# MasterBin-IIAU/UNINEXT

Measured on AMD Instinct MI355X. Metric: frames/sec COCO det+seg R50 1333x800 (MSDeformAttn hot path); MSDeformAttn HBM GB/s, higher is better.
Workload: dtype f32

## Files before the change

include/msda_hip.h:

```cpp
#ifndef MSDA_HIP_H_
#define MSDA_HIP_H_

#include <stddef.h>
#include <stdint.h>

#ifdef __cplusplus
extern "C" {
#endif

#define MSDA_HIP_ABI_VERSION 2

#define MSDA_ERR_NULL_POINTER (-1)
#define MSDA_ERR_BAD_DIMS (-2)
#define MSDA_ERR_TOO_LARGE (-3)
#define MSDA_ERR_BAD_VARIANT (-4)
#define MSDA_ERR_UNSUPPORTED (-5)

int msda_hip_abi_version(void);
const char* msda_hip_last_error(void);

int msda_hip_forward_f32(const float* value, const int64_t* spatial_shapes,
                         const int64_t* level_start_index, const float* sampling_loc,
                         const float* attn_weight, int batch, int spatial_size, int num_heads,
                         int channels, int num_levels, int num_query, int num_point,
                         float* output, void* stream);

int msda_hip_forward_f64(const double* value, const int64_t* spatial_shapes,
                         const int64_t* level_start_index, const double* sampling_loc,
                         const double* attn_weight, int batch, int spatial_size, int num_heads,
                         int channels, int num_levels, int num_query, int num_point,
                         double* output, void* stream);

int msda_hip_backward_f32(const float* grad_output, const float* value,
                          const int64_t* spatial_shapes, const int64_t* level_start_index,
                          const float* sampling_loc, const float* attn_weight, int batch,
                          int spatial_size, int num_heads, int channels, int num_levels,
                          int num_query, int num_point, float* grad_value,
                          float* grad_sampling_loc, float* grad_attn_weight, void* stream);

size_t msda_hip_backward_workspace_bytes(int batch, int spatial_size, int num_heads, int channels, int num_levels,
                                         int num_query, int num_point);
int msda_hip_backward_ws_f32(const float* grad_output, const float* value,
                             const int64_t* spatial_shapes, const int64_t* level_start_index,
                             const float* sampling_loc, const float* attn_weight, int batch,
                             int spatial_size, int num_heads, int channels, int num_levels,
                             int num_query, int num_point, float* grad_value,
                             float* grad_sampling_loc, float* grad_attn_weight, void* workspace,
                             size_t workspace_bytes, void* stream);

int msda_hip_backward_f64(const double* grad_output, const double* value,
                          const int64_t* spatial_shapes, const int64_t* level_start_index,
                          const double* sampling_loc, const double* attn_weight, int batch,
                          int spatial_size, int num_heads, int channels, int num_levels,
                          int num_query, int num_point, double* grad_value,
                          double* grad_sampling_loc, double* grad_attn_weight, void* stream);

int msda_hip_forward_fused_f32(const float* value, const int64_t* spatial_shapes,
                               const int64_t* level_start_index, const float* reference_points, int ref_dim,
                               const float* sampling_offsets, const float* attn_logits, int batch,
                               int spatial_size, int num_heads, int channels, int num_levels, int num_query,
                               int num_point, float* output, void* stream);

int msda_hip_forward_fused_hm_f32(const float* value_head_major, const int64_t* spatial_shapes,
                                  const int64_t* level_start_index, const float* reference_points, int ref_dim,
                                  const float* sampling_offsets, const float* attn_logits, int batch, int spatial_size,
                                  int num_heads, int channels, int num_levels, int num_query, int num_point,
                                  float* output, void* stream);

int msda_hip_prologue_f32(const int64_t* spatial_shapes, const float* reference_points, int ref_dim,
                          const float* sampling_offsets, const float* attn_logits, int batch, int num_heads,
                          int num_levels, int num_query, int num_point, float* sampling_loc, float* attn_weight,
                          void* stream);
int msda_hip_prologue_backward_f32(const int64_t* spatial_shapes, const float* reference_points, int ref_dim,
                                   const float* sampling_offsets, const float* attn_weight,
                                   const float* grad_sampling_loc, const float* grad_attn_weight, int batch,
                                   int num_heads, int num_levels, int num_query, int num_point,
                                   float* grad_sampling_offsets, float* grad_attn_logits,
                                   float* grad_reference_points, void* stream);

int msda_host_forward_f32(const float* value, const int64_t* spatial_shapes, const int64_t* level_start_index,
                          const float* sampling_loc, const float* attn_weight, int batch, int spatial_size,
                          int num_heads, int channels, int num_levels, int num_query, int num_point,
                          float* output, int num_threads);
int msda_host_forward_f64(const double* value, const int64_t* spatial_shapes, const int64_t* level_start_index,
                          const double* sampling_loc, const double* attn_weight, int batch, int spatial_size,
                          int num_heads, int channels, int num_levels, int num_query, int num_point,
                          double* output, int num_threads);
int msda_host_backward_f32(const float* grad_output, const float* value, const int64_t* spatial_shapes,
                           const int64_t* level_start_index, const float* sampling_loc, const float* attn_weight,
                           int batch, int spatial_size, int num_heads, int channels, int num_levels, int num_query,
                           int num_point, float* grad_value, float* grad_sampling_loc, float* grad_attn_weight,
                           int num_threads);
int msda_host_backward_f64(const double* grad_output, const double* value, const int64_t* spatial_shapes,
                           const int64_t* level_start_index, const double* sampling_loc, const double* attn_weight,
                           int batch, int spatial_size, int num_heads, int channels, int num_levels, int num_query,
                           int num_point, double* grad_value, double* grad_sampling_loc, double* grad_attn_weight,
                           int num_threads);

int msda_host_last_num_threads(void);

int msda_hip_set_variant(int which, int variant);
int msda_hip_get_variant(int which);
const char* msda_hip_variant_name(int which, int variant);

const char* msda_hip_last_kernel(int which);

#define MSDA_CTX_GEOMETRY_CHECKED 1u
#define MSDA_CTX_DETERMINISTIC 2u
void msda_hip_set_call_context(int call_site, unsigned flags);
int msda_hip_forward_locality(double* far_fraction);
void msda_hip_reset_call_site(int call_site);

#ifdef __cplusplus
}
#endif
#endif
```

uninext_amd/_lib.py:

```python
import ctypes
import os

_HERE = os.path.dirname(os.path.abspath(__file__))
LIB_PATH = os.environ.get("MSDA_HIP_LIB") or os.path.join(_HERE, "lib", "libmsda_hip.so")

ABI_VERSION = 2

i, p, s, f = ctypes.c_int, ctypes.c_void_p, ctypes.c_char_p, ctypes.c_float
u, z, ll, dp = ctypes.c_uint, ctypes.c_size_t, ctypes.c_longlong, ctypes.POINTER(ctypes.c_double)
_FWD = [p, p, p, p, p, i, i, i, i, i, i, i, p]
_BWD = [p, p, p, p, p, p, i, i, i, i, i, i, i, p, p, p]

_SIGNATURES = {
    "msda_hip.h": {
        "msda_hip_abi_version": (i, []),
        "msda_hip_last_error": (s, []),
        "msda_hip_forward_f32": (i, _FWD + [p]),
        "msda_hip_forward_f64": (i, _FWD + [p]),
        "msda_hip_backward_f32": (i, _BWD + [p]),
        "msda_hip_backward_workspace_bytes": (z, [i, i, i, i, i, i, i]),
        "msda_hip_backward_ws_f32": (i, _BWD + [p, z, p]),
        "msda_hip_backward_f64": (i, _BWD + [p]),
        "msda_hip_forward_fused_f32": (i, [p, p, p, p, i, p, p, i, i, i, i, i, i, i, p, p]),
        "msda_hip_forward_fused_hm_f32": (i, [p, p, p, p, i, p, p, i, i, i, i, i, i, i, p, p]),
        "msda_hip_prologue_f32": (i, [p, p, i, p, p, i, i, i, i, i, p, p, p]),
        "msda_hip_prologue_backward_f32": (i, [p, p, i, p, p, p, p, i, i, i, i, i, p, p, p, p]),
        "msda_host_forward_f32": (i, _FWD + [i]),
        "msda_host_forward_f64": (i, _FWD + [i]),
        "msda_host_backward_f32": (i, _BWD + [i]),
        "msda_host_backward_f64": (i, _BWD + [i]),
        "msda_host_last_num_threads": (i, []),
        "msda_hip_set_variant": (i, [i, i]),
        "msda_hip_get_variant": (i, [i]),
        "msda_hip_variant_name": (s, [i, i]),
        "msda_hip_last_kernel": (s, [i]),
        "msda_hip_set_call_context": (None, [i, u]),
        "msda_hip_forward_locality": (i, [dp]),
        "msda_hip_reset_call_site": (None, [i]),
    },
    "dynmask_hip.h": {
        "dynmask_hip_forward_f32": (i, [p, p, p, p, i, i, i, i, i, i, p, p]),
        "aligned_bilinear_hip_f32": (i, [p, i, i, i, i, p, p]),
        "dynmask_hip_set_variant": (i, [i]),
        "dynmask_hip_last_kernel": (s, []),
        "dynmask_hip_backward_workspace_bytes": (z, [i, i, i]),
        "dynmask_hip_backward_parts": (i, [i, i, i]),
        "dynmask_hip_backward_f32": (i, [p, p, p, p, i, i, i, i, i, i, p, p, p, p, p, z, p]),
        "aligned_bilinear_hip_backward_f32": (i, [p, i, i, i, i, p, p]),
        "qsel_scores_hip_f32": (i, [p, p, p, i, p, p, p, p, p, f, p, ll, p, ll, p, f, i, ll, i, p, p, p]),
        "qsel_boxes_hip_f32": (i, [p, p, p, i, p, p, p, p, p, f, p, ll, p, p, p, p, p, p, i, ll, i, p, p, p]),
        "qsel_hip_last_kernel": (s, []),
        "detpost_scores_hip_f32": (i, [p, p, p, p, i, f, i, i, i, i, p, p, p, p, p]),
        "detpost_nms_hip_f32": (i, [p, p, p, f, i, i, i, p, p, p, p]),
        "detpost_hip_last_kernel": (s, []),
        "maskpost_binarize_hip_f32": (i, [p, p, i, i, i, i, i, i, i, i, i, f, p, p]),
        "maskpost_pack_hip_f32": (i, [p, p, i, i, i, i, p, p, p]),
        "maskpost_nms_hip_u32": (i, [p, p, i, i, f, p, p, p]),
        "maskpost_hip_last_kernel": (s, []),
        "track_hip_state_offset": (z, [i, i, i, i]),
        "track_hip_scores_f32": (i, [p, p, p, p, i, i, i, i, i, i, p, p, p, p]),
        "track_hip_associate_f32": (i, [p, p, p, p, p, p, p, i, i, i, i, i, i, f, f, f, i, i, p, p, p]),
        "track_hip_update_f32": (i, [p, p, p, p, p, p, p, i, i, i, i, i, f, f, i, p]),
        "track_hip_last_kernel": (s, []),
        "qdtrack_hip_state_offset": (z, [i, i, i, i, i]),
        "qdtrack_hip_prepare_f32": (i, [p, i, f, f, f, p, p, p, p]),
        "qdtrack_hip_scores_f32": (i, [p, p, p, p, p, i, i, i, i, i, i, i, i, i, i, i, p, p, p]),
        "qdtrack_hip_associate_f32": (i, [p, p, p, p, p, p, p, i, i, i, i, i, i, i, i, i, i, f, f, f, f, f, i, i, p, p, p]),
        "qdtrack_hip_update_f32": (i, [p, p, p, p, p, p, p, p, i, i, i, i, i, i, i, i, i, i, f, f, i, p]),
        "qdtrack_hip_last_kernel": (s, []),
        "criterion_hip_workspace_bytes": (z, [i, ll, ll]),
        "criterion_hip_last_kernel": (s, []),
        "criterion_hip_token_focal_forward_f32": (i, [p, p, i, p, p, i, f, i, i, i, p, p, z, p]),
        "criterion_hip_token_focal_backward_f32": (i, [p, p, i, p, p, i, f, p, i, i, i, p, p]),
        "criterion_hip_mask_losses_forward_f32": (i, [p, p, p, i, i, i, i, i, i, i, i, f, p, p, p, z, p]),
        "criterion_hip_mask_losses_backward_f32": (i, [p, p, p, p, p, p, i, i, i, i, i, i, i, i, f, p, p]),
        "criterion_hip_box_bitmasks": (i, [p, i, i, i, p, p]),
        "criterion_hip_color_similarity_f32": (i, [p, i, p, p, i, i, i, i, i, p, p, p]),
        "criterion_hip_boxinst_forward_f32": (i, [p] * 7 + [i] * 10 + [f, i] + [p] * 6 + [z, p]),
        "criterion_hip_boxinst_backward_f32": (i, [p] * 13 + [i] * 10 + [f, i, p, p]),
        "encprep_hip_workspace_bytes": (z, [i, p, i]),
        "encprep_hip_masks_u8": (i, [p, i, i, i, p, i, p, p, p, p, p]),
        "encprep_hip_pos_f32": (i, [p, p, p, p, p, i, p, i, i, f, f, p, p, p]),
        "encprep_hip_gn_stats_f32": (i, [p, i, p, i, i, i, p, z, p]),
        "encprep_hip_gn_apply_f32": (i, [p, p, p, p, p, z, i, p, i, i, i, p, p, p, p]),
        "encprep_hip_last_kernel": (s, []),
    },
    "patch_embed_hip.h": {
        "patch_embed_hip_f32": (i, [p, p, p, i, i, i, i, i, i, i, p, p]),
        "patch_embed_hip_packed_weight_bytes": (z, [i, i, i]),
        "patch_embed_hip_pack_weight_f32": (i, [p, i, i, i, p, p]),
        "patch_embed_hip_packed_f32": (i, [p, p, p, i, i, i, i, i, i, i, p, p]),
        "patch_embed_hip_backward_workspace_bytes": (z, [i, i, i, i, i, i]),
        "patch_embed_hip_backward_f32": (i, [p, p, p, i, i, i, i, i, i, i, p, p, p, p, z, p]),
        "patch_embed_hip_convnext_dwconv_ln_f32": (i, [p, p, p, p, p, f, i, i, i, i, p, p]),
        "patch_embed_hip_convnext_scale_residual_f32": (i, [p, p, p, i, i, i, i, p, p]),
        "patch_embed_hip_layernorm_cf_f32": (i, [p, p, p, f, i, i, i, i, p, p]),
        "patch_embed_hip_convnext_last_kernel": (s, []),
        "patch_embed_hip_vit_attn_workspace_bytes": (z, [i, i, i, i, i]),
        "patch_embed_hip_vit_attn_f32": (i, [p, p, p, i, i, i, i, i, f, p, p, z, p]),
        "patch_embed_hip_vit_attn_last_kernel": (s, []),
    },
    "linear_hip.h": {
        "linear_hip_packed_weight_bytes": (z, [i, i]),
        "linear_hip_pack_weight_f32": (i, [p, i, i, p, p]),
        "linear_hip_packed_f32": (i, [p, p, p, p, ll, i, i, p, p]),
        "linear_hip_packed_hm_f32": (i, [p, p, p, p, ll, i, i, i, p, p]),
        "linear_hip_packed_ex_f32": (i, [p, p, p, p, p, ll, i, i, i, p, p]),
        "linear_hip_packed_split_f32": (i, [p, p, p, p, ll, i, i, i, p, p, p]),
        "linear_hip_packed_ln_f32": (i, [p, p, p, p, p, p, f, ll, i, i, p, p]),
        "linear_hip_packed_ffn_f32": (i, [p, p, p, p, p, p, p, p, f, i, ll, i, i, p, p]),
    },
    "layernorm_hip.h": {
        "add_layernorm_hip_f32": (i, [p, p, p, p, f, ll, i, p, p]),
    },
    "lsap_hip.h": {
        "lsap_hip_workspace_bytes": (z, [i, i]),
        "lsap_hip_f32": (i, [p, ll, i, i, p, p, p, p, p]),
        "lsap_hip_batch_f32": (i, [i, p, p, p, p, p, p, p, p, p]),
    },
    "matcher_cost_hip.h": {
        "matcher_cost_hip_f32": (i, [p, p, p, p, p, i, i, i, f, f, f, p, p]),
# ... 19 lines not shown
        "conv3x3_hip_pack_weight_f32": (i, [p, i, i, p, p]),
        "conv3x3_hip_packed_f32": (i, [p, p, p, i, i, i, i, i, i, p, p]),
        "conv3x3_hip_packed_exact_weight_bytes": (z, [i, i]),
        "conv3x3_hip_pack_weight_exact_f32": (i, [p, i, i, p, p]),
        "conv3x3_hip_packed_exact_f32": (i, [p, p, p, i, i, i, i, i, i, p, p]),
        "upsample_add_hip_f32": (i, [p, p, i, i, i, i, i, i, p, p]),
        "conv3x3_hip_packed_exact_dgrad_weight_bytes": (z, [i, i]),
        "conv3x3_hip_pack_weight_exact_dgrad_f32": (i, [p, i, i, p, p]),
        "conv3x3_hip_backward_workspace_bytes": (z, [i, i, i, i, i]),
        "conv3x3_hip_backward_exact_f32": (i, [p, p, p, p, i, i, i, i, i, i, p, p, p, p, z, p]),
    },
}
del i, p, s, f, u, z, ll, dp, _FWD, _BWD

EXPORTS = tuple(_SIGNATURES["msda_hip.h"])
DYNMASK_EXPORTS = tuple(_SIGNATURES["dynmask_hip.h"])
PATCH_EMBED_EXPORTS = tuple(_SIGNATURES["patch_embed_hip.h"])
LINEAR_EXPORTS = tuple(_SIGNATURES["linear_hip.h"])
LAYERNORM_EXPORTS = tuple(_SIGNATURES["layernorm_hip.h"])
LSAP_EXPORTS = tuple(_SIGNATURES["lsap_hip.h"])
MATCHER_COST_EXPORTS = tuple(_SIGNATURES["matcher_cost_hip.h"])
OTA_EXPORTS = tuple(_SIGNATURES["ota_hip.h"])
BIATTN_EXPORTS = tuple(_SIGNATURES["biattn_hip.h"])
CONV3X3_EXPORTS = tuple(_SIGNATURES["conv3x3_hip.h"])

DYNMASK_BWD_MAX_BATCH = 64
BIATTN_MASK_NONE, BIATTN_MASK_INT64, BIATTN_MASK_F32 = 0, 1, 2
BIATTN_MASK_BOOL = 3
DEC_ATTN_HEAD_DIM, DEC_ATTN_MAX_LEN = 32, 65535
BIATTN_HEAD_DIM, BIATTN_MAX_TEXT = 256, 256
VIT_ATTN_HEAD_DIMS = (64, 80)
VIT_ATTN_MAX_SIDE, VIT_ATTN_MAX_TOKENS = 4095, 1 << 20
QSEL_D_MODEL = 256
DETPOST_MAX_CLASSES, DETPOST_MAX_TOKENS, DETPOST_MAX_QUERIES = 4096, 256, 1024
MASKPOST_MAX_WIDTH, MASKPOST_MAX_MASKS, MASKPOST_STRIDES = 8192, 1024, (1, 2, 4, 8)
TRACK_MAX_CAPACITY, TRACK_MAX_DIM, TRACK_MAX_MEMORY_LEN, TRACK_STATE_FIELDS = 4096, 256, 64, 12
QDTRACK_MAX_BACKDROPS, QDTRACK_MAX_BACKDROP_FRAMES, QDTRACK_STATE_FIELDS = 1024, 4, 11
CRITERION_MAX_TOKENS = 256
CRITERION_MASK_NONE, CRITERION_MASK_INT64, CRITERION_MASK_BOOL = 0, 1, 2
CRITERION_TOKEN_FOCAL, CRITERION_MASK_LOSSES, CRITERION_BOXINST = 0, 1, 2
CRITERION_IMAGE_U8, CRITERION_IMAGE_F32 = 0, 1
BOXINST_MAX_DILATION, BOXINST_BAND, BOXINST_LDS_BYTES = 8, 8, 63 * 1024
OTA_MAX_BATCH = 64
REID_MIN_QUERIES, REID_MAX_QUERIES, REID_MAX_DIM, REID_META, REID_STATS = 100, 8192, 512, 5, 6
LSAP_MAX_BATCH = 32
ENCPREP_MAX_LEVELS, ENCPREP_CHANNELS, ENCPREP_GROUPS, ENCPREP_PIXEL_TILE = 8, 256, 32, 32

_lib = None


def load():
    global _lib
    if _lib is not None:
        return _lib
    if not os.path.exists(LIB_PATH):
        raise RuntimeError(
            "MultiScaleDeformableAttention: %s not found. Build it with "
            "`python -c 'import __graft_entry__ as g; g.build()'` or `make -C uninext_amd/csrc` "
            "(hipcc, gfx950). There is no fallback implementation." % LIB_PATH)
    lib = ctypes.CDLL(LIB_PATH)
    for group in _SIGNATURES.values():
        for name, (restype, argtypes) in group.items():
            fn = getattr(lib, name)
            fn.restype, fn.argtypes = restype, argtypes
    got = lib.msda_hip_abi_version()
    if got != ABI_VERSION:
        raise RuntimeError("libmsda_hip.so ABI version %d, binding expects %d: rebuild" % (got, ABI_VERSION))
    _lib = lib
    return lib


def last_error():
    return load().msda_hip_last_error().decode()


def set_variant(which, variant):
    w = {"forward": 0, "backward": 1}[which]
    if isinstance(variant, str):
        variant = variants(which).index(variant)
    if load().msda_hip_set_variant(w, int(variant)) != 0:
        raise ValueError(last_error())


def variants(which):
    w = {"forward": 0, "backward": 1}[which]
    out, k = [], 0
    while True:
        n = load().msda_hip_variant_name(w, k)
        if n is None:
            return out
        out.append(n.decode())
        k += 1


def forward_locality():
    frac = ctypes.c_double(0.0)
    n = load().msda_hip_forward_locality(ctypes.byref(frac))
    return n, frac.value


def last_kernel(which):
    if which == "biattn":
        return load().biattn_hip_last_kernel().decode()
    if which == "dec_attn":
        return load().biattn_hip_self_last_kernel().decode()
    if which == "qsel":
        return load().qsel_hip_last_kernel().decode()
    if which == "detpost":
        return load().detpost_hip_last_kernel().decode()
    if which == "maskpost":
        return load().maskpost_hip_last_kernel().decode()
    if which == "track":
        return load().track_hip_last_kernel().decode()
    if which == "qdtrack":
        return load().qdtrack_hip_last_kernel().decode()
    if which == "encprep":
        return load().encprep_hip_last_kernel().decode()
    if which == "criterion":
        return load().criterion_hip_last_kernel().decode()
    if which == "convnext":
        return load().patch_embed_hip_convnext_last_kernel().decode()
    if which == "vit_attn":
        return load().patch_embed_hip_vit_attn_last_kernel().decode()
    return load().msda_hip_last_kernel({"forward": 0, "backward": 1}[which]).decode()
```

uninext_amd/csrc/msda_capi.hip:

```cpp
#include "../../include/msda_hip.h"

#include <atomic>
#include <cstdio>
#include <cstdlib>
#include <cstring>

#include "launch_glue.hpp"
#include "msda_common.hpp"

namespace {

thread_local char g_err[512] = "";
std::atomic<const char*> g_last_kernel[2] = {{""}, {""}};
std::atomic<int> g_variant[2] = {{-1}, {-1}};

#ifdef MSDA_EXPERIMENTS
#define MSDA_EXP(name) name
constexpr bool kHaveExperiments = true;
#else
#define MSDA_EXP(name) "exp:" name
constexpr bool kHaveExperiments = false;
#endif
constexpr int kNumFwdVariants = msda::kNumVariants, kNumBwdVariants = 9;
const char* const kFwdNames[kNumFwdVariants] = {
// ... 115 lines not shown
                                         int num_query, int num_point) {
  const msda::Dims d{batch, spatial_size, num_heads, channels, num_levels, num_query, num_point};
  if (check_dims(d) || d.N == 0 || d.Lq == 0) return 0;
  return msda::regions_workspace_bytes(d);
}

int msda_hip_backward_ws_f32(const float* grad_output, const float* value, const int64_t* spatial_shapes,
                             const int64_t* level_start_index, const float* sampling_loc, const float* attn_weight,
                             int batch, int spatial_size, int num_heads, int channels, int num_levels, int num_query,
                             int num_point, float* grad_value, float* grad_sampling_loc, float* grad_attn_weight,
                             void* workspace, size_t workspace_bytes, void* stream) {
  const msda::Dims d{batch, spatial_size, num_heads, channels, num_levels, num_query, num_point};
  msda::set_call_workspace(workspace, workspace_bytes);
  return backward_impl<float>(grad_output, value, spatial_shapes, level_start_index, sampling_loc, attn_weight, d,
                              grad_value, grad_sampling_loc, grad_attn_weight, stream);
}

int msda_hip_backward_f64(const double* grad_output, const double* value, const int64_t* spatial_shapes,
                          const int64_t* level_start_index, const double* sampling_loc, const double* attn_weight,
                          int batch, int spatial_size, int num_heads, int channels, int num_levels, int num_query,
                          int num_point, double* grad_value, double* grad_sampling_loc, double* grad_attn_weight,
                          void* stream) {
  const msda::Dims d{batch, spatial_size, num_heads, channels, num_levels, num_query, num_point};
  return backward_impl<double>(grad_output, value, spatial_shapes, level_start_index, sampling_loc, attn_weight, d,
                               grad_value, grad_sampling_loc, grad_attn_weight, stream);
}

static int forward_fused_impl(const float* value, int head_major, const int64_t* spatial_shapes,
                              const int64_t* level_start_index, const float* reference_points, int ref_dim,
                              const float* sampling_offsets, const float* attn_logits, const msda::Dims& d, float* output,
                              void* stream) {
  const ContextScope scope;
  if (int rc = check_dims(d)) return rc;
  if (!msda::fused_forward_ok(d, ref_dim))
    return fail(MSDA_ERR_UNSUPPORTED, "fused forward needs channels == 32, num_levels * num_point == 16, ref_dim 2 or 4");
  if (head_major && !msda::fused_forward_hm_ok(d, ref_dim))
    return fail(MSDA_ERR_UNSUPPORTED, "fused forward on head-major value needs num_levels == num_point == 4 and num_query >= 1024");
  if (d.N == 0 || d.Lq == 0) return 0;
  if (!value || !spatial_shapes || !level_start_index || !reference_points || !sampling_offsets || !attn_logits || !output)
    return fail(MSDA_ERR_NULL_POINTER, "null pointer argument");
  const char* name = "";
  const int rc = msda::launch_forward_fused(current_variant(0), value, head_major, spatial_shapes, level_start_index, reference_points,
                                            ref_dim, sampling_offsets, attn_logits, d, output, (hipStream_t)stream, &name);
  g_last_kernel[0].store(name, std::memory_order_relaxed);
  return finish(rc, "msda_hip_forward_fused");
}

int msda_hip_forward_fused_f32(const float* value, const int64_t* spatial_shapes, const int64_t* level_start_index,
                               const float* reference_points, int ref_dim, const float* sampling_offsets,
                               const float* attn_logits, int batch, int spatial_size, int num_heads, int channels,
                               int num_levels, int num_query, int num_point, float* output, void* stream) {
  const msda::Dims d{batch, spatial_size, num_heads, channels, num_levels, num_query, num_point};
  return forward_fused_impl(value, 0, spatial_shapes, level_start_index, reference_points, ref_dim, sampling_offsets,
                            attn_logits, d, output, stream);
}

int msda_hip_forward_fused_hm_f32(const float* value_head_major, const int64_t* spatial_shapes,
                                  const int64_t* level_start_index, const float* reference_points, int ref_dim,
                                  const float* sampling_offsets, const float* attn_logits, int batch, int spatial_size,
                                  int num_heads, int channels, int num_levels, int num_query, int num_point,
                                  float* output, void* stream) {
  const msda::Dims d{batch, spatial_size, num_heads, channels, num_levels, num_query, num_point};
  return forward_fused_impl(value_head_major, 1, spatial_shapes, level_start_index, reference_points, ref_dim,
                            sampling_offsets, attn_logits, d, output, stream);
}

int msda_hip_set_variant(int which, int variant) {
  if (which < 0 || which > 1 || !variant_available(which, variant))
    return fail(MSDA_ERR_BAD_VARIANT, "unknown kernel variant (or an experiment this build does not carry)");
  g_variant[which].store(variant, std::memory_order_relaxed);
  return 0;
}

int msda_hip_get_variant(int which) { return (which < 0 || which > 1) ? MSDA_ERR_BAD_VARIANT : current_variant(which); }

const char* msda_hip_variant_name(int which, int variant) {
  if (which < 0 || which > 1 || variant < 0 || variant >= num_variants(which)) return nullptr;
  return variant_name(which, variant);
}

int msda_hip_forward_locality(double* far_fraction) { return msda::forward_locality(far_fraction); }
void msda_hip_reset_call_site(int call_site) { msda::reset_call_site(call_site); }

void msda_hip_set_call_context(int call_site, unsigned flags) { msda::set_call_context(call_site, flags); }

const char* msda_hip_last_kernel(int which) {
  return (which < 0 || which > 1) ? "" : g_last_kernel[which].load(std::memory_order_relaxed);
}

}
```

uninext_amd/csrc/msda_common.hpp:

```cpp
#pragma once

#include <hip/hip_runtime.h>
#include <stdint.h>

#include <atomic>
#include <cstdlib>

#include "wave_ops.hpp"

namespace msda {

constexpr int kBlock = 256;
constexpr int kMaxLP = 128;
constexpr int kLevelTableBytes = 3 * kMaxLP * 4;
constexpr uint32_t kOobOffset = 0x80000000u;

typedef unsigned int u32x4 __attribute__((__vector_size__(16)));
typedef float f32x4 __attribute__((__vector_size__(16)));
typedef float f32x2 __attribute__((__vector_size__(8)));

__device__ __forceinline__ f32x4 buffer_load_f32x4(__amdgpu_buffer_rsrc_t rsrc, uint32_t voffset, uint32_t soffset) {
  return __builtin_bit_cast(f32x4, __builtin_amdgcn_raw_buffer_load_b128(rsrc, voffset, soffset, 0));
}

struct Dims {
  int N, S, M, D, L, Lq, P;
};

template <typename T>
struct Sample {
  T lh, lw, hh, hw;
  int h_low, w_low;
  bool in_range;
  bool ok1, ok2, ok3, ok4;
};

template <typename T>
__device__ __forceinline__ Sample<T> make_sample(T loc_w, T loc_h, int H, int W) {
  Sample<T> s;
  const T h_im = loc_h * (T)H - (T)0.5;
  const T w_im = loc_w * (T)W - (T)0.5;
  s.in_range = (h_im > (T)-1) && (w_im > (T)-1) && (h_im < (T)H) && (w_im < (T)W);
  const T hf = floor(h_im), wf = floor(w_im);
  s.h_low = s.in_range ? (int)hf : 0;
  s.w_low = s.in_range ? (int)wf : 0;
  s.lh = h_im - hf;
  s.lw = w_im - wf;
  s.hh = (T)1 - s.lh;
  s.hw = (T)1 - s.lw;
  const bool t = s.in_range && s.h_low >= 0, bt = s.in_range && s.h_low + 1 <= H - 1;
  const bool lf = s.w_low >= 0, rt = s.w_low + 1 <= W - 1;
  s.ok1 = t && lf;
  s.ok2 = t && rt;
  s.ok3 = bt && lf;
  s.ok4 = bt && rt;
  return s;
}

__device__ __forceinline__ void atomic_add(float* p, float v) { unsafeAtomicAdd(p, v); }
__device__ __forceinline__ void atomic_add(double* p, double v) { unsafeAtomicAdd(p, v); }

template <typename T>
int launch_forward(int variant, const T* value, const int64_t* shapes, const int64_t* lsi, const T* loc,
                   const T* attn, const Dims& d, T* out, hipStream_t stream, const char** kernel_name);

template <typename T>
int launch_backward(int variant, const T* grad_out, const T* value, const int64_t* shapes, const int64_t* lsi,
                    const T* loc, const T* attn, const Dims& d, T* grad_value, T* grad_loc, T* grad_attn,
                    hipStream_t stream, const char** kernel_name);

inline int ensure_dynamic_lds(const void* kernel, int bytes, std::atomic<uint64_t>& done) {
  int dev = 0;
  hipError_t e = hipGetDevice(&dev);
  if (e != hipSuccess) return (int)e;
  const uint64_t bit = 1ull << (dev & 63);
  if (done.load(std::memory_order_acquire) & bit) return 0;
  e = hipFuncSetAttribute(kernel, hipFuncAttributeMaxDynamicSharedMemorySize, bytes);
  if (e != hipSuccess) return (int)e;
  done.fetch_or(bit, std::memory_order_release);
  return 0;
}

#ifdef MSDA_EXPERIMENTS
inline int ab_env_int(const char* name, int dflt) {
  const char* e = std::getenv(name);
  return e ? std::atoi(e) : dflt;
}
#else
constexpr int ab_env_int(const char*, int dflt) { return dflt; }
#endif

enum Variant { kAuto = 0, kGeneric = 1, kLaneGroup = 2, kTiled = 3, kTiledL0 = 4, kTiledL0Big = 5, kLaneGroupCL = 6,
               kLaneGroupL3 = 7, kLaneGroupP = 8, kWin = 9, kWin2 = 10, kWin3 = 11, kWin4 = 12, kWinL = 13, kWinP = 14, kNumVariants = 15 };

bool fused_forward_ok(const Dims& d, int ref_dim);
bool fused_forward_hm_ok(const Dims& d, int ref_dim);
int launch_forward_fused(int variant, const float* value, int head_major, const int64_t* shapes, const int64_t* lsi,
                         const float* ref_points, int ref_dim, const float* offsets, const float* logits, const Dims& d,
                         float* out, hipStream_t stream, const char** kernel_name);

bool tiled_backward_ok(const Dims& d);
int launch_backward_tiled(const float* grad_out, const float* value, const int64_t* shapes, const int64_t* lsi,
                          const float* loc, const float* attn, const Dims& d, float* grad_value, float* grad_loc,
                          float* grad_attn, hipStream_t stream);

int launch_backward_tiled_nogv(const float* grad_out, const float* value, const int64_t* shapes, const int64_t* lsi,
                               const float* loc, const float* attn, const Dims& d, float* grad_loc, float* grad_attn,
                               hipStream_t stream);

bool regions_backward_ok(const Dims& d);
bool q_backward_ok(const Dims& d);
int launch_backward_q(const float* grad_out, const float* value, const int64_t* shapes, const int64_t* lsi, const float* loc,
                      const float* attn, const Dims& d, float* grad_loc, float* grad_attn, hipStream_t stream);
size_t regions_workspace_bytes(const Dims& d);
void set_call_workspace(void* p, size_t bytes);
int launch_backward_regions(const float* grad_out, const float* value, const int64_t* shapes, const int64_t* lsi,
                            const float* loc, const float* attn, const Dims& d, float* grad_value, float* grad_loc,
                            float* grad_attn, hipStream_t stream, const char** kernel_name = nullptr);

bool win_backward_ok(const Dims& d);
bool dec_backward_ok(const Dims& d);
int launch_backward_dec(const float* grad_out, const float* value, const int64_t* shapes, const int64_t* lsi, const float* loc,
                        const float* attn, const Dims& d, float* grad_value, float* grad_loc, float* grad_attn, hipStream_t stream);
int launch_backward_win(const float* grad_out, const float* value, const int64_t* shapes, const int64_t* lsi,
                        const float* loc, const float* attn, const Dims& d, float* grad_value, float* grad_loc,
                        float* grad_attn, hipStream_t stream);
bool dst_backward_ok(const Dims& d);
int launch_backward_dst(const float* grad_out, const float* value, const int64_t* shapes, const int64_t* lsi, const float* loc,
                        const float* attn, const Dims& d, float* grad_value, float* grad_loc, float* grad_attn, hipStream_t stream);

bool win_forward_ok(const Dims& d);
bool win_forward_auto(const Dims& d, hipStream_t stream);
bool win2_backward_ok(const Dims& d);
int launch_backward_win2(const float* grad_out, const float* value, const int64_t* shapes, const int64_t* lsi,
                         const float* loc, const float* attn, const Dims& d, float* grad_value, float* grad_loc,
                         float* grad_attn, hipStream_t stream);
int backward_site_choice(const Dims& d);
void set_call_context(int slot, unsigned flags);
void drop_call_context();
int launch_forward_win_fused(const float* value, int head_major, const int64_t* shapes, const int64_t* lsi,
                             const float* ref_points, int ref_dim, const float* offsets, const float* logits, const Dims& d,
                             float* out, hipStream_t stream);
int forward_locality(double* far_fraction);
void reset_call_site(int slot);
int launch_forward_win(const float* value, const int64_t* shapes, const int64_t* lsi, const float* loc, const float* attn,
                       const Dims& d, float* out, hipStream_t stream);

bool winl_forward_ok(const Dims& d);
int launch_forward_winl(const float* value, const int64_t* shapes, const int64_t* lsi, const float* loc, const float* attn,
                        const Dims& d, float* out, hipStream_t stream);

bool winp_forward_ok(const Dims& d);
int launch_forward_winp(const float* value, const int64_t* shapes, const int64_t* lsi, const float* loc, const float* attn,
                        const Dims& d, float* out, hipStream_t stream);

bool win2_forward_ok(const Dims& d);
bool win3_forward_ok(const Dims& d);
bool win4_forward_ok(const Dims& d);
int launch_forward_win4(const float* value, const int64_t* shapes, const int64_t* lsi, const float* loc, const float* attn,
                        const Dims& d, float* out, hipStream_t stream);
int launch_forward_win3(const float* value, const int64_t* shapes, const int64_t* lsi, const float* loc, const float* attn,
                        const Dims& d, float* out, hipStream_t stream);
int launch_forward_win2(const float* value, const int64_t* shapes, const int64_t* lsi, const float* loc, const float* attn,
                        const Dims& d, float* out, hipStream_t stream);

bool tiled_forward_ok(const Dims& d);
int launch_forward_tiled(int flavour, const float* value, const int64_t* shapes, const int64_t* lsi, const float* loc,
                         const float* attn, const Dims& d, float* out, hipStream_t stream);

}
```

uninext_amd/csrc/msda_fwd.hip:

```cpp
#include <type_traits>

#include <cstdlib>

#include "msda_common.hpp"

namespace msda {


template <typename T>
__global__ void __launch_bounds__(kBlock)
msda_fwd_generic(const T* __restrict__ value, const int64_t* __restrict__ shapes,
                 const int64_t* __restrict__ lsi, const T* __restrict__ loc,
                 const T* __restrict__ attn, Dims d, T* __restrict__ out) {
  const int64_t total = (int64_t)d.N * d.Lq * d.M * d.D;
  const int64_t pix_stride = (int64_t)d.M * d.D;
  for (int64_t idx = (int64_t)blockIdx.x * kBlock + threadIdx.x; idx < total;
       idx += (int64_t)gridDim.x * kBlock) {
    const int c = (int)(idx % d.D);
    const int64_t pair = idx / d.D;
    const int m = (int)(pair % d.M);
    const int64_t b = pair / ((int64_t)d.M * d.Lq);
    const T* l_ptr = loc + pair * d.L * d.P * 2;
    const T* a_ptr = attn + pair * d.L * d.P;
    T col = 0;
    for (int l = 0; l < d.L; ++l) {
      const int H = (int)shapes[2 * l], W = (int)shapes[2 * l + 1];
      const T* v_lvl = value + (b * d.S + lsi[l]) * pix_stride + (int64_t)m * d.D + c;
      for (int p = 0; p < d.P; ++p) {
        const Sample<T> s = make_sample<T>(l_ptr[(l * d.P + p) * 2], l_ptr[(l * d.P + p) * 2 + 1], H, W);
        if (!s.in_range) continue;
        const int64_t o1 = ((int64_t)s.h_low * W + s.w_low) * pix_stride;
        const T v1 = s.ok1 ? v_lvl[o1] : (T)0;
        const T v2 = s.ok2 ? v_lvl[o1 + pix_stride] : (T)0;
        const T v3 = s.ok3 ? v_lvl[o1 + (int64_t)W * pix_stride] : (T)0;
        const T v4 = s.ok4 ? v_lvl[o1 + (int64_t)(W + 1) * pix_stride] : (T)0;
        col += (s.hh * s.hw * v1 + s.hh * s.lw * v2 + s.lh * s.hw * v3 + s.lh * s.lw * v4) * a_ptr[l * d.P + p];
      }
    }
    out[idx] = col;
  }
}

__device__ __forceinline__ int rec_pair_stride(int LP) { return LP * 32 + 16; }

template <int G, int LPT>
__global__ void __launch_bounds__(kBlock, 4)
msda_fwd_lanegroup(const float* __restrict__ value, const int64_t* __restrict__ shapes,
                   const int64_t* __restrict__ lsi, const float* __restrict__ loc,
                   const float* __restrict__ attn, Dims d, float* __restrict__ out) {
  constexpr int kPairs = kBlock / G;
  extern __shared__ __attribute__((aligned(16))) char smem[];
  int* smp_H = reinterpret_cast<int*>(smem);
  int* smp_W = smp_H + kMaxLP;
  int* smp_start = smp_W + kMaxLP;
  char* rec_base = smem + kLevelTableBytes;

  const int LP = LPT ? LPT : d.L * d.P;
  const int tid = threadIdx.x;
  if (tid < LP) {
    const int l = tid / d.P;
    smp_H[tid] = (int)shapes[2 * l];
    smp_W[tid] = (int)shapes[2 * l + 1];
    smp_start[tid] = (int)lsi[l];
  }
  __syncthreads();

  const int b = blockIdx.y;
  const int m = blockIdx.x % d.M;
  const int g = tid / G, j = tid % G;
  const int q = (blockIdx.x / d.M) * kPairs + g;
  if (q >= d.Lq) return;

  const int64_t pair = ((int64_t)b * d.Lq + q) * d.M + m;
  const uint32_t pix_bytes = (uint32_t)d.M * d.D * 4u;
  char* rec = rec_base + g * rec_pair_stride(LP);

  auto prepare = [&](int s, float lx, float ly, float a) {
    const int H = smp_H[s], W = smp_W[s];
    const Sample<float> sm = make_sample<float>(lx, ly, H, W);
    const float wa = sm.hh * a, wb = sm.lh * a;
    float4 w;
    w.x = sm.ok1 ? wa * sm.hw : 0.f;
    w.y = sm.ok2 ? wa * sm.lw : 0.f;
    w.z = sm.ok3 ? wb * sm.hw : 0.f;
    w.w = sm.ok4 ? wb * sm.lw : 0.f;
    const uint32_t o1 = (uint32_t)(smp_start[s] + sm.h_low * W + sm.w_low) * pix_bytes;
    u32x4 o;
    o[0] = sm.ok1 ? o1 : kOobOffset;
    o[1] = sm.ok2 ? o1 + pix_bytes : kOobOffset;
    o[2] = sm.ok3 ? o1 + (uint32_t)W * pix_bytes : kOobOffset;
    o[3] = sm.ok4 ? o1 + (uint32_t)(W + 1) * pix_bytes : kOobOffset;
    *reinterpret_cast<float4*>(rec + s * 32) = w;
    *reinterpret_cast<u32x4*>(rec + s * 32 + 16) = o;
  };

  if constexpr (LPT == 2 * G) {
    const float4 lc = *reinterpret_cast<const float4*>(loc + pair * (2 * LPT) + 4 * j);
    const float2 at = *reinterpret_cast<const float2*>(attn + pair * LPT + 2 * j);
    prepare(2 * j, lc.x, lc.y, at.x);
    prepare(2 * j + 1, lc.z, lc.w, at.y);
  } else {
    for (int s = j; s < LP; s += G) {
      const float2 lc = *reinterpret_cast<const float2*>(loc + (pair * LP + s) * 2);
      prepare(s, lc.x, lc.y, attn[pair * LP + s]);
    }
  }
  __builtin_amdgcn_fence(__ATOMIC_RELEASE, "wavefront");
  __builtin_amdgcn_wave_barrier();
  __builtin_amdgcn_fence(__ATOMIC_ACQUIRE, "wavefront");

  const __amdgpu_buffer_rsrc_t rsrc = __builtin_amdgcn_make_buffer_rsrc(
      const_cast<float*>(value) + (int64_t)b * d.S * d.M * d.D, 0, (int)((uint32_t)d.S * pix_bytes), 0x00020000);
  const uint32_t head_off = (uint32_t)m * d.D * 4u;
  const uint32_t lane_off = (uint32_t)j * 16u;
  float4 acc = make_float4(0.f, 0.f, 0.f, 0.f);

  auto gather = [&](int s) {
    const float4 w = *reinterpret_cast<const float4*>(rec + s * 32);
    const u32x4 o = *reinterpret_cast<const u32x4*>(rec + s * 32 + 16);
    const f32x4 r1 = buffer_load_f32x4(rsrc, o[0] + lane_off, head_off);
    const f32x4 r2 = buffer_load_f32x4(rsrc, o[1] + lane_off, head_off);
    const f32x4 r3 = buffer_load_f32x4(rsrc, o[2] + lane_off, head_off);
    const f32x4 r4 = buffer_load_f32x4(rsrc, o[3] + lane_off, head_off);
    acc.x = fmaf(w.w, r4[0], fmaf(w.z, r3[0], fmaf(w.y, r2[0], fmaf(w.x, r1[0], acc.x))));
    acc.y = fmaf(w.w, r4[1], fmaf(w.z, r3[1], fmaf(w.y, r2[1], fmaf(w.x, r1[1], acc.y))));
    acc.z = fmaf(w.w, r4[2], fmaf(w.z, r3[2], fmaf(w.y, r2[2], fmaf(w.x, r1[2], acc.z))));
    acc.w = fmaf(w.w, r4[3], fmaf(w.z, r3[3], fmaf(w.y, r2[3], fmaf(w.x, r1[3], acc.w))));
  };

  if constexpr (LPT != 0) {
#pragma unroll
    for (int s = 0; s < LPT; ++s) gather(s);
  } else {
#pragma unroll 4
    for (int s = 0; s < LP; ++s) gather(s);
  }

  const f32x4 accv = {acc.x, acc.y, acc.z, acc.w};
  __builtin_nontemporal_store(accv, reinterpret_cast<f32x4*>(out + pair * d.D + 4 * j));
}

template <int CTRL>
__device__ __forceinline__ float fdpp(float v) {
  return __int_as_float(__builtin_amdgcn_update_dpp(0, __float_as_int(v), CTRL, 0xF, 0xF, true));
}
__device__ __forceinline__ float group8_max(float v) {
  v = fmaxf(v, fdpp<0xB1>(v));
  v = fmaxf(v, fdpp<0x4E>(v));
  v = fmaxf(v, fdpp<0x141>(v));
  return v;
}
__device__ __forceinline__ float group8_add(float v) {
  v += fdpp<0xB1>(v);
  v += fdpp<0x4E>(v);
  v += fdpp<0x141>(v);
  return v;
}

template <int REFD>
__global__ void __launch_bounds__(kBlock, 4)
msda_fwd_fused(const float* __restrict__ value, const int64_t* __restrict__ shapes,
               const int64_t* __restrict__ lsi, const float* __restrict__ ref_points,
               const float* __restrict__ offsets, const float* __restrict__ logits, Dims d,
               float* __restrict__ out) {
  constexpr int G = 8, LPT = 16, kPairs = kBlock / G;
  extern __shared__ __attribute__((aligned(16))) char smem[];
  int* smp_H = reinterpret_cast<int*>(smem);
  int* smp_W = smp_H + kMaxLP;
  int* smp_start = smp_W + kMaxLP;
  char* rec_base = smem + kLevelTableBytes;
  const int tid = threadIdx.x;
  if (tid < LPT) {
    const int l = tid / d.P;
    smp_H[tid] = (int)shapes[2 * l];
    smp_W[tid] = (int)shapes[2 * l + 1];
    smp_start[tid] = (int)lsi[l];
  }
  __syncthreads();

  const int b = blockIdx.y;
  const int m = blockIdx.x % d.M;
  const int g = tid / G, j = tid % G;
  const int q = (blockIdx.x / d.M) * kPairs + g;
  if (q >= d.Lq) return;

  const int64_t pair = ((int64_t)b * d.Lq + q) * d.M + m;
  const uint32_t pix_bytes = (uint32_t)d.M * 128u;
  char* rec = rec_base + g * (LPT * 32 + 16);

  const float4 off = *reinterpret_cast<const float4*>(offsets + pair * (2 * LPT) + 4 * j);
  const float2 lg = *reinterpret_cast<const float2*>(logits + pair * LPT + 2 * j);
  const int s0 = 2 * j;
  const int lvl = s0 / d.P;
  const int lvl1 = (s0 + 1) / d.P;
  const float* rp = ref_points + ((int64_t)b * d.Lq + q) * d.L * REFD;
  const float mx = group8_max(fmaxf(lg.x, lg.y));
  const float e0 = __expf(lg.x - mx), e1 = __expf(lg.y - mx);
  const float inv = 1.0f / group8_add(e0 + e1);
  const float a0 = e0 * inv, a1 = e1 * inv;

  auto location = [&](int level, float ox, float oy, float& lx, float& ly) {
    if constexpr (REFD == 2) {
      const float2 r = *reinterpret_cast<const float2*>(rp + level * 2);
      lx = r.x + ox / (float)smp_W[level * d.P];
      ly = r.y + oy / (float)smp_H[level * d.P];
    } else {
      const float4 r = *reinterpret_cast<const float4*>(rp + level * 4);
      lx = r.x + ox / (float)d.P * r.z * 0.5f;
      ly = r.y + oy / (float)d.P * r.w * 0.5f;
    }
  };

  auto prepare = [&](int s, float lx, float ly, float a) {
    const int H = smp_H[s], W = smp_W[s];
    const Sample<float> sm = make_sample<float>(lx, ly, H, W);
    const float wa = sm.hh * a, wb = sm.lh * a;
    float4 w;
    w.x = sm.ok1 ? wa * sm.hw : 0.f;
    w.y = sm.ok2 ? wa * sm.lw : 0.f;
    w.z = sm.ok3 ? wb * sm.hw : 0.f;
    w.w = sm.ok4 ? wb * sm.lw : 0.f;
    const uint32_t o1 = (uint32_t)(smp_start[s] + sm.h_low * W + sm.w_low) * pix_bytes;
// ... 198 lines not shown
  auto gather_global = [&](int slot) {
    const float4 w = *reinterpret_cast<const float4*>(rec + slot * 32);
    const u32x4 o = *reinterpret_cast<const u32x4*>(rec + slot * 32 + 16);
    const f32x4 r1 = buffer_load_f32x4(rsrc, o[0] + lane_off, head_off);
    const f32x4 r2 = buffer_load_f32x4(rsrc, o[1] + lane_off, head_off);
    const f32x4 r3 = buffer_load_f32x4(rsrc, o[2] + lane_off, head_off);
    const f32x4 r4 = buffer_load_f32x4(rsrc, o[3] + lane_off, head_off);
#pragma unroll
    for (int c = 0; c < 4; ++c)
      acc[c] = fmaf(w.w, r4[c], fmaf(w.z, r3[c], fmaf(w.y, r2[c], fmaf(w.x, r1[c], acc[c]))));
  };
  auto gather_lds = [&](int slot) {
    typedef const f32x4 __attribute__((address_space(3)))* lp;
    const float4 w = *reinterpret_cast<const float4*>(rec + slot * 32);
    const u32x4 o = *reinterpret_cast<const u32x4*>(rec + slot * 32 + 16);
    const f32x4 r1 = *reinterpret_cast<lp>((uintptr_t)(o[0] + lane_off));
    const f32x4 r2 = *reinterpret_cast<lp>((uintptr_t)(o[1] + lane_off));
    const f32x4 r3 = *reinterpret_cast<lp>((uintptr_t)(o[2] + lane_off));
    const f32x4 r4 = *reinterpret_cast<lp>((uintptr_t)(o[3] + lane_off));
#pragma unroll
    for (int c = 0; c < 4; ++c)
      acc[c] = fmaf(w.w, r4[c], fmaf(w.z, r3[c], fmaf(w.y, r2[c], fmaf(w.x, r1[c], acc[c]))));
  };

  prepare(j, j, lc0.x, lc0.y, at0, false);
  wave_sync();
#pragma unroll
  for (int s = 0; s < 8; ++s) gather_global(s);
  wave_sync();
  prepare(8 + j, j, lc1.x, lc1.y, at1, fits && j >= 4);
  __syncthreads();
#pragma unroll
  for (int s = 0; s < 4; ++s) gather_global(s);
  if (fits) {
#pragma unroll
    for (int s = 4; s < 8; ++s) gather_lds(s);
  } else {
#pragma unroll
    for (int s = 4; s < 8; ++s) gather_global(s);
  }
  if (live) __builtin_nontemporal_store(acc, reinterpret_cast<f32x4*>(out + pair * 32 + 4 * j));
}

static inline bool lg3_ok(const Dims& d) {
  return d.D == 32 && d.P == 4 && d.L == 4 && (int64_t)d.S * d.M * 128 < (int64_t)kOobOffset && d.N <= 65535 &&
         d.Lq >= 1024;
}

template <int REFD>
static int launch_lg3_t(const float* value, const int64_t* shapes, const int64_t* lsi, const float* loc,
                        const float* attn, const float* ref_points, const Dims& d, int head_major, float* out,
                        hipStream_t stream) {
  static std::atomic<uint64_t> lds_opted_in{0};
  if (int rc = ensure_dynamic_lds(reinterpret_cast<const void*>(msda_fwd_lg3<REFD>), kL3LdsBytes, lds_opted_in)) return rc;
  constexpr int kPairs = kL3Threads / 8;
  dim3 grid((unsigned)(d.M * ((d.Lq + kPairs - 1) / kPairs)), (unsigned)d.N);
  hipLaunchKernelGGL(msda_fwd_lg3<REFD>, grid, dim3(kL3Threads), kL3LdsBytes, stream, value, shapes, lsi, loc, attn,
                     ref_points, d, head_major, out);
  return (int)hipGetLastError();
}

static int launch_lg3(const float* value, const int64_t* shapes, const int64_t* lsi, const float* loc,
                      const float* attn, const Dims& d, float* out, hipStream_t stream) {
  return launch_lg3_t<0>(value, shapes, lsi, loc, attn, nullptr, d, 0, out, stream);
}

#ifdef MSDA_EXPERIMENTS
#include "experiments/msda_fwd_lg_variants.inc"
#endif

static inline bool lanegroup_ok(const Dims& d, int* G_out) {
  if (d.D % 4 != 0) return false;
  const int G = d.D / 4;
  if (G < 1 || G > 64 || (G & (G - 1)) != 0) return false;
  if (d.L * d.P > kMaxLP) return false;
  if ((int64_t)d.S * d.M * d.D * 4 >= (int64_t)kOobOffset) return false;
  if (d.N > 65535) return false;
  const int64_t lds = kLevelTableBytes + (int64_t)(kBlock / G) * (d.L * d.P * 32 + 16);
  if (lds > 64 * 1024) return false;
  *G_out = G;
  return true;
}

template <int G, int LPT>
static int launch_lanegroup(const float* value, const int64_t* shapes, const int64_t* lsi, const float* loc,
                            const float* attn, const Dims& d, float* out, hipStream_t stream) {
  constexpr int kPairs = kBlock / G;
  const int LP = d.L * d.P;
  const size_t lds = kLevelTableBytes + (size_t)kPairs * (LP * 32 + 16);
  dim3 grid((unsigned)(d.M * ((d.Lq + kPairs - 1) / kPairs)), (unsigned)d.N);
  hipLaunchKernelGGL((msda_fwd_lanegroup<G, LPT>), grid, dim3(kBlock), lds, stream, value, shapes, lsi, loc, attn,
                     d, out);
  return (int)hipGetLastError();
}

template <>
int launch_forward<float>(int variant, const float* value, const int64_t* shapes, const int64_t* lsi,
                          const float* loc, const float* attn, const Dims& d, float* out, hipStream_t stream,
                          const char** kernel_name) {
  int G = 0;
  const bool lg = lanegroup_ok(d, &G);
#ifdef MSDA_EXPERIMENTS
  const bool tl = tiled_forward_ok(d);
#else
  const bool tl = false;
#endif
  if (variant == kAuto) variant = win_forward_auto(d, stream) ? kWin : (lg3_ok(d) ? kLaneGroupL3 : (lg ? kLaneGroup : kGeneric));
  else drop_call_context();
#ifdef MSDA_EXPERIMENTS
  if (variant == kWinP && !winp_forward_ok(d)) variant = lg3_ok(d) ? kLaneGroupL3 : kLaneGroup;
  if (variant == kWinP) {
    *kernel_name = "msda_fwd_winp";
    return launch_forward_winp(value, shapes, lsi, loc, attn, d, out, stream);
  }
  if (variant == kWinL && !winl_forward_ok(d)) variant = lg3_ok(d) ? kLaneGroupL3 : kLaneGroup;
  if (variant == kWinL) {
    *kernel_name = "msda_fwd_winl";
    return launch_forward_winl(value, shapes, lsi, loc, attn, d, out, stream);
  }
  if (variant == kWin4 && !win4_forward_ok(d)) variant = lg3_ok(d) ? kLaneGroupL3 : kLaneGroup;
  if (variant == kWin4) {
    *kernel_name = "msda_fwd_win4";
    return launch_forward_win4(value, shapes, lsi, loc, attn, d, out, stream);
  }
  if (variant == kWin3 && !win3_forward_ok(d)) variant = lg3_ok(d) ? kLaneGroupL3 : kLaneGroup;
  if (variant == kWin3) {
    *kernel_name = "msda_fwd_win3";
    return launch_forward_win3(value, shapes, lsi, loc, attn, d, out, stream);
  }
  if (variant == kWin2 && !win2_forward_ok(d)) variant = lg3_ok(d) ? kLaneGroupL3 : kLaneGroup;
  if (variant == kWin2) {
    *kernel_name = "msda_fwd_win2";
    return launch_forward_win2(value, shapes, lsi, loc, attn, d, out, stream);
  }
#endif
  if (variant == kWin && !win_forward_ok(d)) variant = lg3_ok(d) ? kLaneGroupL3 : kLaneGroup;
  if (variant == kWin) {
    *kernel_name = "msda_fwd_win";
    return launch_forward_win(value, shapes, lsi, loc, attn, d, out, stream);
  }
  if (variant == kLaneGroupL3 && !lg3_ok(d)) variant = kLaneGroup;
  if (variant == kLaneGroupL3) {
    *kernel_name = "msda_fwd_lg3";
    return launch_lg3(value, shapes, lsi, loc, attn, d, out, stream);
  }
#ifdef MSDA_EXPERIMENTS
  if (variant == kLaneGroupP && !lg3_ok(d)) variant = kLaneGroup;
  if (variant == kLaneGroupP) {
    *kernel_name = "msda_fwd_lgp";
    return launch_lgp(value, shapes, lsi, loc, attn, d, out, stream);
  }
  if (variant == kLaneGroupCL && !lgcl_ok(d)) variant = kLaneGroup;
  if (variant == kLaneGroupCL) {
    *kernel_name = "msda_fwd_lgcl";
    return launch_lgcl(value, shapes, lsi, loc, attn, d, out, stream);
  }
#endif
  if (variant >= kTiled && !tl) variant = lg ? kLaneGroup : kGeneric;
  if (variant == kLaneGroup && !lg) variant = kGeneric;
#ifdef MSDA_EXPERIMENTS
  if (variant >= kTiled) {
    *kernel_name = "msda_fwd_tiled";
    return launch_forward_tiled(variant - kTiled, value, shapes, lsi, loc, attn, d, out, stream);
  }
#endif
  if (variant == kLaneGroup) {
    const int LP = d.L * d.P;
    *kernel_name = "msda_fwd_lanegroup";
    switch (G) {
      case 1: return launch_lanegroup<1, 0>(value, shapes, lsi, loc, attn, d, out, stream);
      case 2: return launch_lanegroup<2, 0>(value, shapes, lsi, loc, attn, d, out, stream);
// ... 31 lines not shown
```

Baseline: 3926.

## Specialize lanegroup forward for L=4,P=4,D=32 with software-pipelined gathers

Adds a dedicated msda_fwd_lanegroup<8,16> specialization that keeps level shapes in registers instead of an LDS table. It maps each lane to one level and issues buffer loads three samples ahead of the FMA accumulation, with a flattened pair-indexed grid and launch bounds of 8. The goal is to hide gather latency and cut LDS table setup and occupancy limits on the common Deformable-DETR config. The generic template drops its compile-time LPT paths, and a runtime switch can force the generic path. The cost is higher register pressure from the prefetch buffers, and the specialization hardcodes D=32.

```diff
diff --git a/include/msda_hip.h b/include/msda_hip.h
--- a/include/msda_hip.h
+++ b/include/msda_hip.h
@@ -105,6 +105,8 @@
 
 const char* msda_hip_last_kernel(int which);
 
+void msda_hip_set_lanegroup_general(int on);
+
 #define MSDA_CTX_GEOMETRY_CHECKED 1u
 #define MSDA_CTX_DETERMINISTIC 2u
 void msda_hip_set_call_context(int call_site, unsigned flags);
diff --git a/uninext_amd/_lib.py b/uninext_amd/_lib.py
--- a/uninext_amd/_lib.py
+++ b/uninext_amd/_lib.py
@@ -37,6 +37,7 @@
         "msda_hip_set_call_context": (None, [i, u]),
         "msda_hip_forward_locality": (i, [dp]),
         "msda_hip_reset_call_site": (None, [i]),
+        "msda_hip_set_lanegroup_general": (None, [i]),
     },
     "dynmask_hip.h": {
         "dynmask_hip_forward_f32": (i, [p, p, p, p, i, i, i, i, i, i, p, p]),
@@ -222,6 +223,10 @@
         raise ValueError(last_error())
 
 
+def set_lanegroup_general(on):
+    load().msda_hip_set_lanegroup_general(1 if on else 0)
+
+
 def variants(which):
     w = {"forward": 0, "backward": 1}[which]
     out, k = [], 0
diff --git a/uninext_amd/csrc/msda_capi.hip b/uninext_amd/csrc/msda_capi.hip
--- a/uninext_amd/csrc/msda_capi.hip
+++ b/uninext_amd/csrc/msda_capi.hip
@@ -221,6 +221,8 @@
 int msda_hip_forward_locality(double* far_fraction) { return msda::forward_locality(far_fraction); }
 void msda_hip_reset_call_site(int call_site) { msda::reset_call_site(call_site); }
 
+void msda_hip_set_lanegroup_general(int on) { msda::set_lanegroup_general(on); }
+
 void msda_hip_set_call_context(int call_site, unsigned flags) { msda::set_call_context(call_site, flags); }
 
 const char* msda_hip_last_kernel(int which) {
diff --git a/uninext_amd/csrc/msda_common.hpp b/uninext_amd/csrc/msda_common.hpp
--- a/uninext_amd/csrc/msda_common.hpp
+++ b/uninext_amd/csrc/msda_common.hpp
@@ -93,6 +93,8 @@
 enum Variant { kAuto = 0, kGeneric = 1, kLaneGroup = 2, kTiled = 3, kTiledL0 = 4, kTiledL0Big = 5, kLaneGroupCL = 6,
                kLaneGroupL3 = 7, kLaneGroupP = 8, kWin = 9, kWin2 = 10, kWin3 = 11, kWin4 = 12, kWinL = 13, kWinP = 14, kNumVariants = 15 };
 
+void set_lanegroup_general(int on);
+
 bool fused_forward_ok(const Dims& d, int ref_dim);
 bool fused_forward_hm_ok(const Dims& d, int ref_dim);
 int launch_forward_fused(int variant, const float* value, int head_major, const int64_t* shapes, const int64_t* lsi,
diff --git a/uninext_amd/csrc/msda_fwd.hip b/uninext_amd/csrc/msda_fwd.hip
--- a/uninext_amd/csrc/msda_fwd.hip
+++ b/uninext_amd/csrc/msda_fwd.hip
@@ -48,6 +48,7 @@
 msda_fwd_lanegroup(const float* __restrict__ value, const int64_t* __restrict__ shapes,
                    const int64_t* __restrict__ lsi, const float* __restrict__ loc,
                    const float* __restrict__ attn, Dims d, float* __restrict__ out) {
+  static_assert(LPT == 0, "only <8, 16> has a compile-time L * P");
   constexpr int kPairs = kBlock / G;
   extern __shared__ __attribute__((aligned(16))) char smem[];
   int* smp_H = reinterpret_cast<int*>(smem);
@@ -55,7 +56,7 @@
   int* smp_start = smp_W + kMaxLP;
   char* rec_base = smem + kLevelTableBytes;
 
-  const int LP = LPT ? LPT : d.L * d.P;
+  const int LP = d.L * d.P;
   const int tid = threadIdx.x;
   if (tid < LP) {
     const int l = tid / d.P;
@@ -94,16 +95,9 @@
     *reinterpret_cast<u32x4*>(rec + s * 32 + 16) = o;
   };
 
-  if constexpr (LPT == 2 * G) {
-    const float4 lc = *reinterpret_cast<const float4*>(loc + pair * (2 * LPT) + 4 * j);
-    const float2 at = *reinterpret_cast<const float2*>(attn + pair * LPT + 2 * j);
-    prepare(2 * j, lc.x, lc.y, at.x);
-    prepare(2 * j + 1, lc.z, lc.w, at.y);
-  } else {
-    for (int s = j; s < LP; s += G) {
-      const float2 lc = *reinterpret_cast<const float2*>(loc + (pair * LP + s) * 2);
-      prepare(s, lc.x, lc.y, attn[pair * LP + s]);
-    }
+  for (int s = j; s < LP; s += G) {
+    const float2 lc = *reinterpret_cast<const float2*>(loc + (pair * LP + s) * 2);
+    prepare(s, lc.x, lc.y, attn[pair * LP + s]);
   }
   __builtin_amdgcn_fence(__ATOMIC_RELEASE, "wavefront");
   __builtin_amdgcn_wave_barrier();
@@ -128,16 +122,89 @@
     acc.w = fmaf(w.w, r4[3], fmaf(w.z, r3[3], fmaf(w.y, r2[3], fmaf(w.x, r1[3], acc.w))));
   };
 
-  if constexpr (LPT != 0) {
-#pragma unroll
-    for (int s = 0; s < LPT; ++s) gather(s);
-  } else {
 #pragma unroll 4
-    for (int s = 0; s < LP; ++s) gather(s);
-  }
+  for (int s = 0; s < LP; ++s) gather(s);
 
   const f32x4 accv = {acc.x, acc.y, acc.z, acc.w};
   __builtin_nontemporal_store(accv, reinterpret_cast<f32x4*>(out + pair * d.D + 4 * j));
+}
+
+template <>
+__global__ void __launch_bounds__(kBlock, 8)
+msda_fwd_lanegroup<8, 16>(const float* __restrict__ value, const int64_t* __restrict__ shapes,
+                          const int64_t* __restrict__ lsi, const float* __restrict__ loc,
+                          const float* __restrict__ attn, Dims d, float* __restrict__ out) {
+  constexpr int G = 8, LPT = 16, kPairs = kBlock / G, kRecPair = LPT * 32 + 16, kDepth = 3;
+  extern __shared__ __attribute__((aligned(16))) char smem[];
+  const int tid = threadIdx.x;
+  const int g = tid / G, j = tid % G;
+  const int b = blockIdx.y;
+
+  int lvH[4], lvW[4], lvS[4];
+#pragma unroll
+  for (int l = 0; l < 4; ++l) {
+    lvH[l] = (int)shapes[2 * l];
+    lvW[l] = (int)shapes[2 * l + 1];
+    lvS[l] = (int)lsi[l];
+  }
+  const int l = j >> 1;
+  const int H = l == 0 ? lvH[0] : l == 1 ? lvH[1] : l == 2 ? lvH[2] : lvH[3];
+  const int W = l == 0 ? lvW[0] : l == 1 ? lvW[1] : l == 2 ? lvW[2] : lvW[3];
+  const int start = l == 0 ? lvS[0] : l == 1 ? lvS[1] : l == 2 ? lvS[2] : lvS[3];
+
+  const int p = (int)blockIdx.x * kPairs + g;
+  if (p >= d.Lq * d.M) return;
+  const int m = p % d.M;
+  const int64_t pair = (int64_t)b * d.Lq * d.M + p;
+  const uint32_t pix_bytes = (uint32_t)d.M * 128u;
+  char* rec = smem + g * kRecPair;
+
+  const float4 lc = *reinterpret_cast<const float4*>(loc + pair * (2 * LPT) + 4 * j);
+  const float2 at = *reinterpret_cast<const float2*>(attn + pair * LPT + 2 * j);
+  auto prepare = [&](int s, float lx, float ly, float a) {
+    const Sample<float> sm = make_sample<float>(lx, ly, H, W);
+    const float wa = sm.hh * a, wb = sm.lh * a;
+    float4 w;
+    w.x = sm.ok1 ? wa * sm.hw : 0.f;
+    w.y = sm.ok2 ? wa * sm.lw : 0.f;
+    w.z = sm.ok3 ? wb * sm.hw : 0.f;
+    w.w = sm.ok4 ? wb * sm.lw : 0.f;
+    const uint32_t o1 = (uint32_t)(start + sm.h_low * W + sm.w_low) * pix_bytes;
+    u32x4 o;
+    o[0] = sm.ok1 ? o1 : kOobOffset;
+    o[1] = sm.ok2 ? o1 + pix_bytes : kOobOffset;
+    o[2] = sm.ok3 ? o1 + (uint32_t)W * pix_bytes : kOobOffset;
+    o[3] = sm.ok4 ? o1 + (uint32_t)(W + 1) * pix_bytes : kOobOffset;
+    *reinterpret_cast<float4*>(rec + s * 32) = w;
+    *reinterpret_cast<u32x4*>(rec + s * 32 + 16) = o;
+  };
+  prepare(2 * j, lc.x, lc.y, at.x);
+  prepare(2 * j + 1, lc.z, lc.w, at.y);
+  __builtin_amdgcn_fence(__ATOMIC_RELEASE, "wavefront");
+  __builtin_amdgcn_wave_barrier();
+  __builtin_amdgcn_fence(__ATOMIC_ACQUIRE, "wavefront");
+
+  const __amdgpu_buffer_rsrc_t rsrc = __builtin_amdgcn_make_buffer_rsrc(
+      const_cast<float*>(value) + (int64_t)b * d.S * d.M * 32, 0, (int)((uint32_t)d.S * pix_bytes), 0x00020000);
+  const uint32_t lane_off = (uint32_t)m * 128u + (uint32_t)j * 16u;
+  f32x4 r[LPT][4];
+  auto issue = [&](int s) {
+    const u32x4 o = *reinterpret_cast<const u32x4*>(rec + s * 32 + 16);
+#pragma unroll
+    for (int c = 0; c < 4; ++c) r[s][c] = buffer_load_f32x4(rsrc, o[c] + lane_off, 0u);
+  };
+  f32x4 acc = {0.f, 0.f, 0.f, 0.f};
+#pragma unroll
+  for (int s = 0; s < kDepth; ++s) issue(s);
+#pragma unroll
+  for (int s = 0; s < LPT; ++s) {
+    const float4 w = *reinterpret_cast<const float4*>(rec + s * 32);
+#pragma unroll
+    for (int c = 0; c < 4; ++c)
+      acc[c] = fmaf(w.w, r[s][3][c], fmaf(w.z, r[s][2][c], fmaf(w.y, r[s][1][c], fmaf(w.x, r[s][0][c], acc[c]))));
+    if (s + kDepth < LPT) issue(s + kDepth);
+  }
+  __builtin_nontemporal_store(acc, reinterpret_cast<f32x4*>(out + pair * 32 + 4 * j));
 }
 
 template <int CTRL>
@@ -502,11 +569,22 @@
   return true;
 }
 
+static std::atomic<int> g_lanegroup_general{0};
+void set_lanegroup_general(int on) { g_lanegroup_general.store(on, std::memory_order_relaxed); }
+
 template <int G, int LPT>
 static int launch_lanegroup(const float* value, const int64_t* shapes, const int64_t* lsi, const float* loc,
                             const float* attn, const Dims& d, float* out, hipStream_t stream) {
   constexpr int kPairs = kBlock / G;
   const int LP = d.L * d.P;
+  if constexpr (LPT == 16) {
+    if (d.L != 4 || d.P != 4 || g_lanegroup_general.load(std::memory_order_relaxed))
+      return launch_lanegroup<8, 0>(value, shapes, lsi, loc, attn, d, out, stream);
+    dim3 grid((unsigned)(((int64_t)d.Lq * d.M + kPairs - 1) / kPairs), (unsigned)d.N);
+    hipLaunchKernelGGL((msda_fwd_lanegroup<8, 16>), grid, dim3(kBlock), (size_t)kPairs * (16 * 32 + 16), stream, value,
+                       shapes, lsi, loc, attn, d, out);
+    return (int)hipGetLastError();
+  }
   const size_t lds = kLevelTableBytes + (size_t)kPairs * (LP * 32 + 16);
   dim3 grid((unsigned)(d.M * ((d.Lq + kPairs - 1) / kPairs)), (unsigned)d.N);
   hipLaunchKernelGGL((msda_fwd_lanegroup<G, LPT>), grid, dim3(kBlock), lds, stream, value, shapes, lsi, loc, attn,
```

Measured after the change: 3992 (median of 6 runs). +1.7%, better.
